# beautifulv0id/Convex-2D-GPU-Collision-Detection

Hardware: AMD Instinct MI355X
Metric: sat_pair_tests_per_s (higher is better)
Workload: dtype f32

## Files before the change

convex-2d-gpu-collision-detection_amd/csrc/c2d_math.hpp:

```cpp
#pragma once

#include <hip/hip_runtime.h>
#include <stdint.h>

namespace c2d {

#define C2D_DEV __device__ __forceinline__

C2D_DEV float fma_(float a, float b, float c) { return __builtin_fmaf(a, b, c); }

C2D_DEV float log_(float u)
{
    uint32_t t = __float_as_uint(u) - 0x3f2aaaabu;
    int32_t e = (int32_t)t >> 23;
    float m = __uint_as_float((t & 0x007fffffu) + 0x3f2aaaabu);
    float f = m - 1.0f;
    float q = -0x1.04cba2p-3f;
    q = fma_(q, f, 0x1.19bbe2p-3f);
    q = fma_(q, f, -0x1.f483fap-4f);
    q = fma_(q, f, 0x1.1fd494p-3f);
    q = fma_(q, f, -0x1.55913ep-3f);
    q = fma_(q, f, 0x1.99bffep-3f);
    q = fma_(q, f, -0x1.ffff28p-3f);
    q = fma_(q, f, 0x1.55552cp-2f);
    q = fma_(q, f, -0x1.000000p-1f);
    float s = f * f;
    float r = fma_(s, q, f);
    return fma_((float)e, 0x1.62e430p-1f, r);
}

C2D_DEV float sqrt_normal_range(float x)
{
    const float s = __builtin_amdgcn_sqrtf(x);
    const float s_dn = __uint_as_float(__float_as_uint(s) - 1u);
    const float s_up = __uint_as_float(__float_as_uint(s) + 1u);
    const float r_dn = fma_(-s_dn, s, x);
    const float r_up = fma_(-s_up, s, x);
    float r = r_dn <= 0.0f ? s_dn : s;
    r = r_up > 0.0f ? s_up : r;
    return r;
}

C2D_DEV void quadrant_rotate(int q, float sn, float cs, float& s_out, float& c_out)
{
    float a = (q & 1) ? cs : sn;
    float b = (q & 1) ? sn : cs;
    uint32_t s_sign = ((uint32_t)q & 2u) << 30;
    uint32_t c_sign = (((uint32_t)q + 1u) & 2u) << 30;
    s_out = __uint_as_float(__float_as_uint(a) ^ s_sign);
    c_out = __uint_as_float(__float_as_uint(b) ^ c_sign);
}

C2D_DEV void sincos_(float x, float& s_out, float& c_out)
{
    float k = __builtin_rintf(x * 0x1.45f306p-1f);
    float r = fma_(k, -0x1.920000p+0f, x);
    r = fma_(k, -0x1.fb4000p-12f, r);
    r = fma_(k, -0x1.4442d2p-24f, r);
    float z = r * r;
    float sp = 0x1.6dac7ap-19f;
    sp = fma_(sp, z, -0x1.a01376p-13f);
    sp = fma_(sp, z, 0x1.11110ep-7f);
    sp = fma_(sp, z, -0x1.555556p-3f);
    float sn = fma_(z * r, sp, r);
    float cp = -0x1.2476a8p-22f;
    cp = fma_(cp, z, 0x1.a012bap-16f);
    cp = fma_(cp, z, -0x1.6c16bcp-10f);
    cp = fma_(cp, z, 0x1.555556p-5f);
    cp = fma_(cp, z, -0x1.000000p-1f);
    float cs = fma_(z, cp, 1.0f);
    float kc = __builtin_amdgcn_fmed3f(k, -1073741824.0f, 1073741824.0f);
    int q = (int)kc;
    quadrant_rotate(q, sn, cs, s_out, c_out);
}

C2D_DEV void sincos_u32(uint32_t y, float& s_out, float& c_out)
{
    int q = (int)(y >> 30);
    uint32_t fr = y & 0x3fffffffu;
    bool swap = fr > 0x20000000u;
    fr = swap ? 0x40000000u - fr : fr;
    float x = (float)(int32_t)fr * 0x1p-30f;
    float z = x * x;
    float p = 0x1.4bb0a6p-13f;
    p = fma_(p, z, -0x1.32ca4ap-8f);
    p = fma_(p, z, 0x1.466bbap-4f);
    p = fma_(p, z, -0x1.4abbcep-1f);
    p = fma_(p, z, 0x1.921fb6p+0f);
    float sn = p * x;
    float c = 0x1.d99986p-11f;
    c = fma_(c, z, -0x1.55c4e6p-6f);
    c = fma_(c, z, 0x1.03c1dap-2f);
    c = fma_(c, z, -0x1.3bd3ccp+0f);
    c = fma_(c, z, 1.0f);
    float sn2 = swap ? c : sn;
    float cs2 = swap ? sn : c;
    quadrant_rotate(q, sn2, cs2, s_out, c_out);
}

struct U4 { uint32_t x, y, z, w; };

C2D_DEV U4 philox4x32_10(uint32_t c0, uint32_t c1, uint32_t c2, uint32_t c3, uint32_t k0, uint32_t k1)
{
#pragma unroll
    for (int round = 0; round < 10; round++) {
        uint64_t p0 = (uint64_t)0xD2511F53u * c0;
        uint64_t p1 = (uint64_t)0xCD9E8D57u * c2;
        uint32_t n0 = __builtin_amdgcn_bitop3_b32((uint32_t)(p1 >> 32), c1, k0, 0x96);
        uint32_t n1 = (uint32_t)p1;
        uint32_t n2 = __builtin_amdgcn_bitop3_b32((uint32_t)(p0 >> 32), c3, k1, 0x96);
        uint32_t n3 = (uint32_t)p0;
        c0 = n0; c1 = n1; c2 = n2; c3 = n3;
        k0 += 0x9E3779B9u;
        k1 += 0xBB67AE85u;
    }
    return U4{c0, c1, c2, c3};
}

C2D_DEV U4 philox_block(uint64_t seed, uint64_t scene, uint64_t sample, uint32_t j)
{
    uint64_t blk = 2 * sample + j;
    return philox4x32_10((uint32_t)blk, (uint32_t)(blk >> 32), (uint32_t)scene, (uint32_t)(scene >> 32),
                         (uint32_t)seed, (uint32_t)(seed >> 32));
}

C2D_DEV U4 philox_draw_block(uint64_t seed, uint64_t scene, uint64_t group, uint32_t b)
{
    uint64_t blk = 8 * group + b;
    return philox4x32_10((uint32_t)blk, (uint32_t)(blk >> 32), (uint32_t)scene, (uint32_t)(scene >> 32),
                         (uint32_t)seed, (uint32_t)(seed >> 32));
}

C2D_DEV uint32_t u4_word(const U4& v, int j) { return j == 0 ? v.x : (j == 1 ? v.y : (j == 2 ? v.z : v.w)); }

C2D_DEV void box_muller(uint32_t x, uint32_t y, float& n0, float& n1)
{
    float u = fma_((float)x, 0x1p-32f, 0x1p-33f);
    float rad = sqrt_normal_range(-2.0f * log_(u));
    float sn, cs;
    sincos_u32(y, sn, cs);
    n0 = sn * rad;
    n1 = cs * rad;
}


#ifndef C2D_FMAD
#define C2D_FMAD 0
#endif
C2D_DEV float dot2(float a, float x, float b, float y)
{
#if C2D_FMAD == 1
    return fma_(a, x, b * y);
#elif C2D_FMAD == 2
    return fma_(b, y, a * x);
#else
    return a * x + b * y;
#endif
}

C2D_DEV void rect_from_half_extents(float hx, float hy, float c, float s, float dx, float dy, float (&r)[8])
{
#if C2D_FMAD == 1
    float b = s * hy, q = c * hy;
    float t1 = fma_(c, hx, b), t2 = fma_(c, hx, -b), t3 = fma_(s, hx, q), t4 = fma_(s, hx, -q);
#elif C2D_FMAD == 2
    float a = c * hx, p = s * hx;
    float t1 = fma_(s, hy, a), t2 = fma_(-s, hy, a), t3 = fma_(c, hy, p), t4 = fma_(-c, hy, p);
#else
    float a = c * hx, b = s * hy, p = s * hx, q = c * hy;
    float t1 = a + b, t2 = a - b, t3 = p + q, t4 = p - q;
#endif
    r[0] = dx - t2;
    r[1] = dy - t3;
    r[2] = t1 + dx;
    r[3] = t4 + dy;
    r[4] = t2 + dx;
    r[5] = t3 + dy;
    r[6] = dx - t1;
    r[7] = dy - t4;
}

C2D_DEV void poly_minmax(float nx, float ny, float x, float y, float& mn, float& mx)
{
    const float p = nx * x + ny * y;
    mn = __builtin_fminf(mn, p);
    mx = __builtin_fmaxf(mx, p);
}

C2D_DEV float min4(float a, float b, float c, float d) { return __builtin_fminf(__builtin_fminf(a, b), __builtin_fminf(c, d)); }
C2D_DEV float max4(float a, float b, float c, float d) { return __builtin_fmaxf(__builtin_fmaxf(a, b), __builtin_fmaxf(c, d)); }

C2D_DEV bool first_projections_ordered(float p1_first, float p2_first) { return !__builtin_isunordered(p1_first, p2_first); }

C2D_DEV bool axis_separates(float ax, float ay, const float (&r1)[8], const float (&r2)[8])
{
    float p10 = dot2(ax, r1[0], ay, r1[1]), p11 = dot2(ax, r1[2], ay, r1[3]);
    float p12 = dot2(ax, r1[4], ay, r1[5]), p13 = dot2(ax, r1[6], ay, r1[7]);
    float p20 = dot2(ax, r2[0], ay, r2[1]), p21 = dot2(ax, r2[2], ay, r2[3]);
    float p22 = dot2(ax, r2[4], ay, r2[5]), p23 = dot2(ax, r2[6], ay, r2[7]);
    float min1 = min4(p10, p11, p12, p13), max1 = max4(p10, p11, p12, p13);
    float min2 = min4(p20, p21, p22, p23), max2 = max4(p20, p21, p22, p23);
    return ((max1 < min2) || (max2 < min1)) && first_projections_ordered(p10, p20);
}

C2D_DEV bool rect_collide(const float (&r1)[8], const float (&r2)[8])
{
    bool sep = false;
#pragma unroll
    for (int i = 0; i < 4; i++) {
        float ax = r1[(2 * i + 2) & 7] - r1[2 * i];
        float ay = r1[(2 * i + 3) & 7] - r1[2 * i + 1];
        sep |= axis_separates(ax, ay, r1, r2);
    }
#pragma unroll
    for (int i = 0; i < 4; i++) {
        float ax = r2[(2 * i + 2) & 7] - r2[2 * i];
        float ay = r2[(2 * i + 3) & 7] - r2[2 * i + 1];
        sep |= axis_separates(ax, ay, r1, r2);
    }
    return !sep;
}

C2D_DEV bool rect_collide_certified(const float (&r1)[8], const float (&r2)[8], bool& thin)
{
    float cmax = __builtin_fabsf(r1[0]);
#pragma unroll
    for (int k = 1; k < 8; k++) cmax = __builtin_fmaxf(cmax, __builtin_fabsf(r1[k]));
#pragma unroll
    for (int k = 0; k < 8; k++) cmax = __builtin_fmaxf(cmax, __builtin_fabsf(r2[k]));
    const float c2 = (2.0f + 0x1p-7f) * cmax, c3 = (8.0f + 0x1p-5f) * 0x1p-24f * cmax;
    bool sep = false, uneasy = !(cmax < 0x1p61f);
#pragma unroll
    for (int which = 0; which < 2; which++) {
        const float (&r)[8] = which == 0 ? r1 : r2;
#pragma unroll
        for (int i = 0; i < 2; i++) {
            const float ax = r[2 * i + 2] - r[2 * i], ay = r[2 * i + 3] - r[2 * i + 1];
            const float bx = r[(2 * i + 6) & 7] - r[2 * i + 4], by = r[(2 * i + 7) & 7] - r[2 * i + 5];
            const float p10 = dot2(ax, r1[0], ay, r1[1]), p11 = dot2(ax, r1[2], ay, r1[3]);
            const float p12 = dot2(ax, r1[4], ay, r1[5]), p13 = dot2(ax, r1[6], ay, r1[7]);
            const float p20 = dot2(ax, r2[0], ay, r2[1]), p21 = dot2(ax, r2[2], ay, r2[3]);
            const float p22 = dot2(ax, r2[4], ay, r2[5]), p23 = dot2(ax, r2[6], ay, r2[7]);
            const float min1 = min4(p10, p11, p12, p13), max1 = max4(p10, p11, p12, p13);
            const float min2 = min4(p20, p21, p22, p23), max2 = max4(p20, p21, p22, p23);
            sep |= ((max1 < min2) || (max2 < min1)) && first_projections_ordered(p10, p20);
            const float need = fma_(__builtin_fabsf(ax) + __builtin_fabsf(ay), c3, (__builtin_fabsf(ax + bx) + __builtin_fabsf(ay + by)) * c2) + 1e-36f;
            uneasy |= !((max2 - min1 >= need) && (max1 - min2 >= need));
        }
    }
    thin = !sep && uneasy;
    return !sep;
}

}
```

convex-2d-gpu-collision-detection_amd/csrc/c2d_sat.hip:

```cpp
#include "c2d_internal.hpp"
#include "c2d_math.hpp"
#include "c2d_count.hpp"
#include "c2d_wave.hpp"

namespace c2d {

struct Planes16 { const float* p[16]; };
struct Planes10 { const float* p[10]; };
struct Planes8 { float* p[8]; };

constexpr int kBlock = 256;
constexpr int kWideBlock = 64;
constexpr int kMaxBlocks = kMaxGrid;


template <int PAIRS, class Build>
C2D_DEV uint32_t collide_pairs(Build build)
{
    uint32_t bits = 0;
    bool any_thin = false;
#pragma unroll
    for (int e = 0; e < PAIRS; e++) {
        float r1[8], r2[8];
        build(e, Plain{}, r1, r2);
        bool thin;
        bits |= (rect_collide_certified(r1, r2, thin) ? 1u : 0u) << e;
        any_thin |= thin;
    }
    if (__ballot(any_thin) != 0ull) {
        bits = 0;
#pragma unroll
        for (int e = 0; e < PAIRS; e++) {
            float r1[8], r2[8];
            build(e, Laundered{}, r1, r2);
            bits |= (rect_collide(r1, r2) ? 1u : 0u) << e;
        }
    }
    return bits;
}

C2D_DEV uint32_t bits_to_bytes4(uint32_t b) { return (b & 1u) | ((b & 2u) << 7) | ((b & 4u) << 14) | ((b & 8u) << 21); }

template <int VEC, int BLOCK>
__global__ __launch_bounds__(BLOCK, (VEC == 4 ? 5 : 1)) void sat_rect_verts_kernel(Planes16 P, size_t first, size_t n_groups,
                                                                uint8_t* __restrict__ out,
                                                                unsigned long long* __restrict__ d_count, CountWs words)
{
    uint32_t my_count = 0;
    const size_t stride = (size_t)gridDim.x * BLOCK;
    for (size_t g = (size_t)blockIdx.x * BLOCK + threadIdx.x; g < n_groups; g += stride) {
        if constexpr (VEC == 4) {
            f32x4 v[16];
#pragma unroll
            for (int k = 0; k < 16; k++) v[k] = __builtin_nontemporal_load(reinterpret_cast<const f32x4*>(P.p[k]) + g);
            const uint32_t packed = bits_to_bytes4(collide_pairs<4>([&v](int e, auto how, float (&r1)[8], float (&r2)[8]) {
#pragma unroll
                for (int k = 0; k < 8; k++) {
                    r1[k] = launder(v[k][e], how);
                    r2[k] = launder(v[8 + k][e], how);
                }
            }));
            my_count += (uint32_t)__popc(packed);
            __builtin_nontemporal_store(packed, reinterpret_cast<uint32_t*>(out) + g);
        } else {
            const size_t i = first + g;
            float r1[8], r2[8];
#pragma unroll
            for (int k = 0; k < 8; k++) {
                r1[k] = P.p[k][i];
                r2[k] = P.p[8 + k][i];
            }
            uint32_t c = rect_collide(r1, r2) ? 1u : 0u;
            out[i] = (uint8_t)c;
            my_count += c;
        }
    }
    if (d_count) wave_count_arrive(my_count, d_count, words);
}

__global__ __launch_bounds__(64) void sat_rect_verts_mask4_kernel(Planes16 P, size_t n_groups, unsigned long long* __restrict__ mask,
                                                                  unsigned long long* __restrict__ d_count,
                                                                  CountWs words)
{
    const uint32_t lane = threadIdx.x;
    const size_t g = (size_t)blockIdx.x * 64 + lane;
    uint32_t nib = 0;
    if (g < n_groups) {
        f32x4 v[16];
#pragma unroll
        for (int k = 0; k < 16; k++) v[k] = __builtin_nontemporal_load(reinterpret_cast<const f32x4*>(P.p[k]) + g);
        nib = collide_pairs<4>([&v](int e, auto how, float (&r1)[8], float (&r2)[8]) {
#pragma unroll
            for (int k = 0; k < 8; k++) {
                r1[k] = launder(v[k][e], how);
                r2[k] = launder(v[8 + k][e], how);
            }
        });
    }
    const uint32_t sh = 4u * (lane & 15u);
    uint32_t lo = sh < 32u ? nib << sh : 0u, hi = sh >= 32u ? nib << (sh - 32u) : 0u;
#pragma unroll
    for (int off = 1; off < 16; off <<= 1) {
        lo |= (uint32_t)__shfl_xor((int)lo, off, 64);
        hi |= (uint32_t)__shfl_xor((int)hi, off, 64);
    }
    if ((lane & 15u) == 0 && g < n_groups) __builtin_nontemporal_store(((unsigned long long)hi << 32) | lo, mask + ((size_t)blockIdx.x * 4 + (lane >> 4)));
    if (d_count) wave_count_arrive((uint32_t)__popc(nib), d_count, words);
}

__global__ __launch_bounds__(kBlock) void sat_rect_verts_mask1_kernel(Planes16 P, size_t first, size_t n, unsigned long long* __restrict__ mask,
                                                                      unsigned long long* __restrict__ d_count,
                                                                      CountWs words)
{
    uint32_t my_count = 0;
    const size_t stride = (size_t)gridDim.x * kBlock;
    const size_t n_round = (n + 63) / 64 * 64;
    for (size_t i = first + (size_t)blockIdx.x * kBlock + threadIdx.x; i < n_round; i += stride) {
        uint32_t c = 0;
        if (i < n) {
            float r1[8], r2[8];
#pragma unroll
            for (int k = 0; k < 8; k++) {
                r1[k] = P.p[k][i];
                r2[k] = P.p[8 + k][i];
            }
            c = rect_collide(r1, r2) ? 1u : 0u;
        }
        const unsigned long long b = __ballot(c != 0);
        if ((threadIdx.x & 63) == 0) mask[i >> 6] = b;
        my_count += c;
    }
    if (d_count) wave_count_arrive(my_count, d_count, words);
}

template <bool OUT16>
__global__ __launch_bounds__(64) void sat_rect_aos_kernel(const float* __restrict__ r1s, const float* __restrict__ r2s,
                                                         size_t n, uint8_t* __restrict__ out,
                                                         unsigned long long* __restrict__ d_count,
                                                         CountWs words)
{
    constexpr int kChunks = 256;
    __shared__ __attribute__((aligned(16))) f32x4 tile[2][kChunks];
    const int lane = threadIdx.x;
    uint32_t my_count = 0;
    const size_t n_tiles = (n + 127) / 128;
    for (size_t t = blockIdx.x; t < n_tiles; t += gridDim.x) {
        const size_t p0 = t * 128;
        const size_t chunks = (n - p0 < 128 ? n - p0 : 128) * 2;
        const f32x4* a = reinterpret_cast<const f32x4*>(r1s) + 2 * p0;
        const f32x4* b = reinterpret_cast<const f32x4*>(r2s) + 2 * p0;
        const f32x4 zero = {0.f, 0.f, 0.f, 0.f};
        f32x4 va[4], vb[4];
#pragma unroll
        for (int k = 0; k < 4; k++) {
            const size_t c = (size_t)(64 * k + lane);
            va[k] = c < chunks ? __builtin_nontemporal_load(a + c) : zero;
            vb[k] = c < chunks ? __builtin_nontemporal_load(b + c) : zero;
        }
#pragma unroll
        for (int k = 0; k < 4; k++) {
            tile[0][64 * k + lane] = va[k];
            tile[1][64 * k + lane] = vb[k];
        }
        wave_lds_sync();
        f32x4 pa[4], pb[4];
#pragma unroll
        for (int c = 0; c < 4; c++) {
            pa[c] = tile[0][4 * lane + c];
            pb[c] = tile[1][4 * lane + c];
        }
        const uint32_t bits = collide_pairs<2>([&pa, &pb](int e, auto how, float (&r1)[8], float (&r2)[8]) {
#pragma unroll
            for (int k = 0; k < 8; k++) {
                r1[k] = launder(pa[2 * e + k / 4][k % 4], how);
                r2[k] = launder(pb[2 * e + k / 4][k % 4], how);
            }
        });
        const uint32_t packed = (bits & 1u) | ((bits & 2u) << 7);
        const size_t i = p0 + 2 * (size_t)lane;
        if (i + 1 < n) {
            if constexpr (OUT16) {
                *reinterpret_cast<uint16_t*>(out + i) = (uint16_t)packed;
            } else {
                out[i] = (uint8_t)(packed & 1u);
                out[i + 1] = (uint8_t)(packed >> 8);
            }
            my_count += (uint32_t)__popc(packed);
        } else if (i < n) {
            out[i] = (uint8_t)(packed & 1u);
            my_count += packed & 1u;
        }
        wave_lds_sync();
    }
    if (d_count) wave_count_arrive(my_count, d_count, words);
}

C2D_DEV bool pose_pair_closed_form(const float (&v)[10], bool& thin)
{
    float s1, c1, s2, c2;
    sincos_(v[4], s1, c1);
    sincos_(v[9], s2, c2);
    const float hw = __builtin_fabsf(v[2] / 2), hh = __builtin_fabsf(v[3] / 2), hx = __builtin_fabsf(v[7] / 2), hy = __builtin_fabsf(v[8] / 2);
    const float q1 = fma_(c1, c2, s1 * s2), q2 = fma_(c1, s2, -(s1 * c2));
    const float ex = v[5] - v[0], ey = v[6] - v[1];
    const float t1 = fma_(c1, ex, s1 * ey), t2 = fma_(c1, ey, -(s1 * ex));
    const float t3 = fma_(c2, ex, s2 * ey), t4 = fma_(c2, ey, -(s2 * ex));
    const float a1 = __builtin_fabsf(q1), a2 = __builtin_fabsf(q2);
    const float g1 = __builtin_fabsf(t1) - fma_(hx, a1, fma_(hy, a2, hw));
    const float g2 = __builtin_fabsf(t2) - fma_(hx, a2, fma_(hy, a1, hh));
    const float g3 = __builtin_fabsf(t3) - fma_(hw, a1, fma_(hh, a2, hx));
    const float g4 = __builtin_fabsf(t4) - fma_(hw, a2, fma_(hh, a1, hy));
    const float C = __builtin_fmaxf(__builtin_fmaxf(__builtin_fabsf(v[0]), __builtin_fabsf(v[1])) + (hw + hh),
                                    __builtin_fmaxf(__builtin_fabsf(v[5]), __builtin_fabsf(v[6])) + (hx + hy)) * (1.0f + 0x1p-10f);
    const float uc = (0x1p-24f * (1.0f + 0x1p-10f)) * C, k64 = 64.0f * uc, k20 = (20.0f * uc) * C;
    const float z1 = g1 * hw, z2 = g2 * hh, z3 = g3 * hx, z4 = g4 * hy;
    const float m1 = fma_(k64, hw, k20), m2 = fma_(k64, hh, k20), m3 = fma_(k64, hx, k20), m4 = fma_(k64, hy, k20);
    const float over = __builtin_fmaxf(__builtin_fmaxf(z1 - m1, z2 - m2), __builtin_fmaxf(z3 - m3, z4 - m4));
    const float under = __builtin_fmaxf(__builtin_fmaxf(z1 + m1, z2 + m2), __builtin_fmaxf(z3 + m3, z4 + m4));
    const float all = (g1 + g2) + (g3 + g4);
    const float hmin = __builtin_fminf(__builtin_fminf(hw, hh), __builtin_fminf(hx, hy));
    const bool regular = (C < 1e15f) & (hmin >= 1e-12f) & (__builtin_fabsf(all) < 1e37f);
    const bool sep = over > 0.0f, col = under < 0.0f;
    thin = !(regular & (sep | col));
    return col;
}

C2D_DEV void pose_pair_rects(const float (&v)[10], float (&r1)[8], float (&r2)[8])
{
    float s, c;
    sincos_(v[4], s, c);
    rect_from_half_extents(v[2] / 2, v[3] / 2, c, s, v[0], v[1], r1);
    sincos_(v[9], s, c);
    rect_from_half_extents(v[7] / 2, v[8] / 2, c, s, v[5], v[6], r2);
}

C2D_DEV uint32_t pose_pair_collides(const float (&v)[10])
{
    float r1[8], r2[8];
    pose_pair_rects(v, r1, r2);
    return rect_collide(r1, r2) ? 1u : 0u;
}

template <int VEC, int BLOCK>
__global__ __launch_bounds__(BLOCK, (VEC == 4 ? 5 : 1)) void sat_rect_pose_kernel(Planes10 P, size_t first, size_t n_groups,
                                                              uint8_t* __restrict__ out,
                                                              unsigned long long* __restrict__ d_count,
                                                              CountWs words)
{
    uint32_t my_count = 0;
    const size_t stride = (size_t)gridDim.x * BLOCK;
    for (size_t g = (size_t)blockIdx.x * BLOCK + threadIdx.x; g < n_groups; g += stride) {
        if constexpr (VEC == 4) {
            f32x4 q[10];
#pragma unroll
            for (int k = 0; k < 10; k++) q[k] = __builtin_nontemporal_load(reinterpret_cast<const f32x4*>(P.p[k]) + g);
            uint32_t bits = 0;
#pragma unroll
            for (int e = 0; e < 4; e++) {
                float v[10];
#pragma unroll
                for (int k = 0; k < 10; k++) v[k] = q[k][e];
                bool thin;
                uint32_t hit = pose_pair_closed_form(v, thin) ? 1u : 0u;
                if (__ballot(thin) != 0ull) {
                    hit = collide_pairs<1>([&q, e](int, auto, float (&r1)[8], float (&r2)[8]) {
                        float w[10];
#pragma unroll
                        for (int k = 0; k < 10; k++) w[k] = launder(q[k][e], Laundered{});
                        pose_pair_rects(w, r1, r2);
                    });
                }
                bits |= hit << e;
            }
            const uint32_t packed = bits_to_bytes4(bits);
            my_count += (uint32_t)__popc(packed);
            __builtin_nontemporal_store(packed, reinterpret_cast<uint32_t*>(out) + g);
        } else {
            const size_t i = first + g;
            float v[10];
#pragma unroll
            for (int k = 0; k < 10; k++) v[k] = P.p[k][i];
            const uint32_t hit = pose_pair_collides(v);
            out[i] = (uint8_t)hit;
            my_count += hit;
        }
    }
    if (d_count) wave_count_arrive(my_count, d_count, words);
}

__global__ __launch_bounds__(kBlock) void rects_from_poses_kernel(const float* __restrict__ cx, const float* __restrict__ cy,
                                                                  const float* __restrict__ w, const float* __restrict__ h,
                                                                  const float* __restrict__ th, size_t n, Planes8 O)
{
    const size_t stride = (size_t)gridDim.x * kBlock;
    for (size_t i = (size_t)blockIdx.x * kBlock + threadIdx.x; i < n; i += stride) {
        float r[8], s, c;
        sincos_(th[i], s, c);
        rect_from_half_extents(w[i] / 2, h[i] / 2, c, s, cx[i], cy[i], r);
#pragma unroll
        for (int k = 0; k < 8; k++) O.p[k][i] = r[k];
    }
}

__global__ __launch_bounds__(kWideBlock) void rects_from_poses4_kernel(const float* __restrict__ cx, const float* __restrict__ cy,
                                                                       const float* __restrict__ w, const float* __restrict__ h,
                                                                       const float* __restrict__ th, size_t n_groups, Planes8 O)
{
    const size_t stride = (size_t)gridDim.x * kWideBlock;
    for (size_t g = (size_t)blockIdx.x * kWideBlock + threadIdx.x; g < n_groups; g += stride) {
        const f32x4 vcx = __builtin_nontemporal_load(reinterpret_cast<const f32x4*>(cx) + g);
        const f32x4 vcy = __builtin_nontemporal_load(reinterpret_cast<const f32x4*>(cy) + g);
        const f32x4 vw = __builtin_nontemporal_load(reinterpret_cast<const f32x4*>(w) + g);
        const f32x4 vh = __builtin_nontemporal_load(reinterpret_cast<const f32x4*>(h) + g);
        const f32x4 vt = __builtin_nontemporal_load(reinterpret_cast<const f32x4*>(th) + g);
        f32x4 o[8];
#pragma unroll
        for (int e = 0; e < 4; e++) {
            float r[8], s, c;
            sincos_(vt[e], s, c);
            rect_from_half_extents(vw[e] / 2, vh[e] / 2, c, s, vcx[e], vcy[e], r);
#pragma unroll
            for (int k = 0; k < 8; k++) o[k][e] = r[k];
        }
#pragma unroll
        for (int k = 0; k < 8; k++) __builtin_nontemporal_store(o[k], reinterpret_cast<f32x4*>(O.p[k]) + g);
    }
}

static inline bool aligned_to(const void* p, size_t a) { return (reinterpret_cast<uintptr_t>(p) & (a - 1)) == 0; }

}

using namespace c2d;

extern "C" {

int c2d_rects_from_poses(c2d_ctx* ctx, const float* d_cx, const float* d_cy, const float* d_w, const float* d_h,
                         const float* d_theta, size_t n, float* const d_out_planes[8], c2d_stream stream)
{
    if (!ctx) return C2D_ERR_INVALID_ARG;
    if (n == 0) return C2D_OK;
    if (!d_cx || !d_cy || !d_w || !d_h || !d_theta || !d_out_planes) return fail_arg(ctx, "c2d_rects_from_poses: NULL plane");
    Planes8 O;
    for (int k = 0; k < 8; k++) {
        if (!d_out_planes[k]) return fail_arg(ctx, "c2d_rects_from_poses: NULL output plane");
        O.p[k] = d_out_planes[k];
    }
    DeviceGuard g(ctx->device);
    bool wide = aligned_to(d_cx, 16) && aligned_to(d_cy, 16) && aligned_to(d_w, 16) && aligned_to(d_h, 16) && aligned_to(d_theta, 16);
    for (int k = 0; k < 8; k++) wide = wide && aligned_to(O.p[k], 16);
    const size_t n4 = wide ? n / 4 : 0;
    if (n4) {
        hipLaunchKernelGGL(rects_from_poses4_kernel, dim3(grid_for(n4, kWideBlock, kMaxBlocks)), dim3(kWideBlock), 0, (hipStream_t)stream, d_cx, d_cy,
                           d_w, d_h, d_theta, n4, O);
        C2D_LAUNCH_CHECK(ctx);
    }
    const size_t rest = n - 4 * n4;
    if (rest) {
        Planes8 T;
        for (int k = 0; k < 8; k++) T.p[k] = O.p[k] + 4 * n4;
        hipLaunchKernelGGL(rects_from_poses_kernel, dim3(grid_for(rest, kBlock, ctx->prop.multiProcessorCount * 8)), dim3(kBlock), 0,
                           (hipStream_t)stream, d_cx + 4 * n4, d_cy + 4 * n4, d_w + 4 * n4, d_h + 4 * n4, d_theta + 4 * n4, rest, T);
        C2D_LAUNCH_CHECK(ctx);
    }
    return C2D_OK;
}

int c2d_sat_rect_pairs_verts(c2d_ctx* ctx, const float* const d_planes[16], size_t n, uint8_t* d_out,
                             unsigned long long* d_count, c2d_stream stream)
{
    if (!ctx) return C2D_ERR_INVALID_ARG;
    if (n == 0) return C2D_OK;
    if (!d_planes || !d_out) return fail_arg(ctx, "c2d_sat_rect_pairs_verts: NULL argument");
    Planes16 P;
    bool wide = aligned_to(d_out, 4);
    for (int k = 0; k < 16; k++) {
        if (!d_planes[k]) return fail_arg(ctx, "c2d_sat_rect_pairs_verts: NULL plane");
        P.p[k] = d_planes[k];
        wide = wide && aligned_to(d_planes[k], 16);
    }
    DeviceGuard g(ctx->device);
    hipStream_t s = (hipStream_t)stream;
    if (int rc = workspace_acquire(ctx, s, d_count != nullptr)) return rc;
    const size_t n4 = wide ? n / 4 : 0;
    if (n4) {
        const int grid = grid_for(n4, kWideBlock, kMaxBlocks);
        hipLaunchKernelGGL((sat_rect_verts_kernel<4, kWideBlock>), dim3(grid), dim3(kWideBlock), 0, s, P, (size_t)0, n4, d_out,
                           d_count, workspace_count_ticket(ctx, s, (size_t)grid * (kWideBlock / 64), d_count != nullptr));
        C2D_LAUNCH_CHECK(ctx);
    }
    const size_t rest = n - 4 * n4;
    if (rest) {
        const int grid = grid_for(rest, kBlock, kMaxBlocks);
        hipLaunchKernelGGL((sat_rect_verts_kernel<1, kBlock>), dim3(grid), dim3(kBlock), 0, s, P, 4 * n4, rest, d_out, d_count,
                           workspace_count_ticket(ctx, s, (size_t)grid * (kBlock / 64), d_count != nullptr));
        C2D_LAUNCH_CHECK(ctx);
    }
    return C2D_OK;
}

int c2d_sat_rect_pairs_verts_mask(c2d_ctx* ctx, const float* const d_planes[16], size_t n, unsigned long long* d_mask,
                                  unsigned long long* d_count, c2d_stream stream)
{
    if (!ctx) return C2D_ERR_INVALID_ARG;
    if (n == 0) return C2D_OK;
    if (!d_planes || !d_mask) return fail_arg(ctx, "c2d_sat_rect_pairs_verts_mask: NULL argument");
    if (!aligned_to(d_mask, 8)) return fail_arg(ctx, "c2d_sat_rect_pairs_verts_mask: the mask must be 8-byte aligned");
    Planes16 P;
    bool wide = true;
    for (int k = 0; k < 16; k++) {
        if (!d_planes[k]) return fail_arg(ctx, "c2d_sat_rect_pairs_verts_mask: NULL plane");
        P.p[k] = d_planes[k];
        wide = wide && aligned_to(d_planes[k], 16);
    }
    DeviceGuard g(ctx->device);
    hipStream_t s = (hipStream_t)stream;
    if (int rc = workspace_acquire(ctx, s, d_count != nullptr)) return rc;
    size_t done = 0;
    while (wide && n - done >= 64) {
        size_t words_left = (n - done) / 64;
        if (words_left > (size_t)kMaxBlocks * 4) words_left = (size_t)kMaxBlocks * 4;
        Planes16 Q;
        for (int k = 0; k < 16; k++) Q.p[k] = P.p[k] + done;
        const size_t groups = words_left * 16;
        hipLaunchKernelGGL(sat_rect_verts_mask4_kernel, dim3((unsigned)((groups + 63) / 64)), dim3(64), 0, s, Q, groups, d_mask + done / 64, d_count,
                           workspace_count_ticket(ctx, s, (groups + 63) / 64, d_count != nullptr));
        C2D_LAUNCH_CHECK(ctx);
        done += words_left * 64;
    }
    if (done < n) {
        const int grid = grid_for(n - done, kBlock, kMaxBlocks);
        hipLaunchKernelGGL(sat_rect_verts_mask1_kernel, dim3(grid), dim3(kBlock), 0, s, P, done, n, d_mask, d_count,
                           workspace_count_ticket(ctx, s, (size_t)grid * (kBlock / 64), d_count != nullptr));
        C2D_LAUNCH_CHECK(ctx);
    }
    return C2D_OK;
}

int c2d_sat_rect_pairs_aos(c2d_ctx* ctx, const float* d_r1, const float* d_r2, size_t n, uint8_t* d_out,
                           unsigned long long* d_count, c2d_stream stream)
{
    if (!ctx) return C2D_ERR_INVALID_ARG;
    if (n == 0) return C2D_OK;
    if (!d_r1 || !d_r2 || !d_out) return fail_arg(ctx, "c2d_sat_rect_pairs_aos: NULL argument");
    if (!aligned_to(d_r1, 16) || !aligned_to(d_r2, 16)) return fail_arg(ctx, "c2d_sat_rect_pairs_aos: rectangle arrays must be 16-byte aligned");
    DeviceGuard g(ctx->device);
    if (int rc = workspace_acquire(ctx, (hipStream_t)stream, d_count != nullptr)) return rc;
    const int grid = grid_for(n, 128, kMaxBlocks);
    const CountWs ws = workspace_count_ticket(ctx, (hipStream_t)stream, (size_t)grid, d_count != nullptr);
    if (aligned_to(d_out, 2))
        hipLaunchKernelGGL(sat_rect_aos_kernel<true>, dim3(grid), dim3(64), 0, (hipStream_t)stream, d_r1, d_r2, n, d_out, d_count, ws);
    else
        hipLaunchKernelGGL(sat_rect_aos_kernel<false>, dim3(grid), dim3(64), 0, (hipStream_t)stream, d_r1, d_r2, n, d_out, d_count, ws);
    C2D_LAUNCH_CHECK(ctx);
    return C2D_OK;
}

int c2d_sat_rect_pairs_pose(c2d_ctx* ctx, const float* const d_pose_planes[10], size_t n, uint8_t* d_out,
                            unsigned long long* d_count, c2d_stream stream)
{
    if (!ctx) return C2D_ERR_INVALID_ARG;
    if (n == 0) return C2D_OK;
    if (!d_pose_planes || !d_out) return fail_arg(ctx, "c2d_sat_rect_pairs_pose: NULL argument");
    Planes10 P;
    bool wide = aligned_to(d_out, 4);
    for (int k = 0; k < 10; k++) {
        if (!d_pose_planes[k]) return fail_arg(ctx, "c2d_sat_rect_pairs_pose: NULL plane");
        P.p[k] = d_pose_planes[k];
        wide = wide && aligned_to(d_pose_planes[k], 16);
    }
    DeviceGuard g(ctx->device);
    hipStream_t s = (hipStream_t)stream;
    if (int rc = workspace_acquire(ctx, s, d_count != nullptr)) return rc;
    const size_t n4 = wide ? n / 4 : 0;
    if (n4) {
        const int grid = grid_for(n4, kWideBlock, kMaxBlocks);
        hipLaunchKernelGGL((sat_rect_pose_kernel<4, kWideBlock>), dim3(grid), dim3(kWideBlock), 0, s, P, (size_t)0, n4, d_out,
                           d_count, workspace_count_ticket(ctx, s, (size_t)grid * (kWideBlock / 64), d_count != nullptr));
        C2D_LAUNCH_CHECK(ctx);
    }
    const size_t rest = n - 4 * n4;
    if (rest) {
        const int grid = grid_for(rest, kBlock, kMaxBlocks);
        hipLaunchKernelGGL((sat_rect_pose_kernel<1, kBlock>), dim3(grid), dim3(kBlock), 0, s, P, 4 * n4, rest, d_out, d_count,
                           workspace_count_ticket(ctx, s, (size_t)grid * (kBlock / 64), d_count != nullptr));
        C2D_LAUNCH_CHECK(ctx);
    }
    return C2D_OK;
}

}
```

Before: 95.60 billion.

## Replace certified SAT projection test with center-gap formulation and simplify pose fallback

Replaces the per-axis min/max projection certified test with a rectangle gap test. It uses center differences, edge-vector dot products and rounding-error margins, so each axis needs far fewer dot products and min/max operations. The pose kernel fallback now calls pose_pair_collides directly on laundered inputs instead of going through collide_pairs. The new error bounds must remain sound, and they may send more pairs down the thin/exact fallback path.

```diff
diff --git a/convex-2d-gpu-collision-detection_amd/csrc/c2d_math.hpp b/convex-2d-gpu-collision-detection_amd/csrc/c2d_math.hpp
--- a/convex-2d-gpu-collision-detection_amd/csrc/c2d_math.hpp
+++ b/convex-2d-gpu-collision-detection_amd/csrc/c2d_math.hpp
@@ -221,35 +221,39 @@
     return !sep;
 }
 
-C2D_DEV bool rect_collide_certified(const float (&r1)[8], const float (&r2)[8], bool& thin)
-{
-    float cmax = __builtin_fabsf(r1[0]);
-#pragma unroll
-    for (int k = 1; k < 8; k++) cmax = __builtin_fmaxf(cmax, __builtin_fabsf(r1[k]));
-#pragma unroll
-    for (int k = 0; k < 8; k++) cmax = __builtin_fmaxf(cmax, __builtin_fabsf(r2[k]));
-    const float c2 = (2.0f + 0x1p-7f) * cmax, c3 = (8.0f + 0x1p-5f) * 0x1p-24f * cmax;
-    bool sep = false, uneasy = !(cmax < 0x1p61f);
-#pragma unroll
-    for (int which = 0; which < 2; which++) {
-        const float (&r)[8] = which == 0 ? r1 : r2;
-#pragma unroll
-        for (int i = 0; i < 2; i++) {
-            const float ax = r[2 * i + 2] - r[2 * i], ay = r[2 * i + 3] - r[2 * i + 1];
-            const float bx = r[(2 * i + 6) & 7] - r[2 * i + 4], by = r[(2 * i + 7) & 7] - r[2 * i + 5];
-            const float p10 = dot2(ax, r1[0], ay, r1[1]), p11 = dot2(ax, r1[2], ay, r1[3]);
-            const float p12 = dot2(ax, r1[4], ay, r1[5]), p13 = dot2(ax, r1[6], ay, r1[7]);
-            const float p20 = dot2(ax, r2[0], ay, r2[1]), p21 = dot2(ax, r2[2], ay, r2[3]);
-            const float p22 = dot2(ax, r2[4], ay, r2[5]), p23 = dot2(ax, r2[6], ay, r2[7]);
-            const float min1 = min4(p10, p11, p12, p13), max1 = max4(p10, p11, p12, p13);
-            const float min2 = min4(p20, p21, p22, p23), max2 = max4(p20, p21, p22, p23);
-            sep |= ((max1 < min2) || (max2 < min1)) && first_projections_ordered(p10, p20);
-            const float need = fma_(__builtin_fabsf(ax) + __builtin_fabsf(ay), c3, (__builtin_fabsf(ax + bx) + __builtin_fabsf(ay + by)) * c2) + 1e-36f;
-            uneasy |= !((max2 - min1 >= need) && (max1 - min2 >= need));
-        }
-    }
-    thin = !sep && uneasy;
-    return !sep;
-}
-
-}
+
+C2D_DEV float dotf(float px, float py, float qx, float qy) { return fma_(px, qx, py * qy); }
+
+C2D_DEV bool rect_gap_certified(const float (&r1)[8], const float (&r2)[8], bool& thin)
+{
+    const float a1x = r1[2] - r1[0], a1y = r1[3] - r1[1], b1x = r1[6] - r1[0], b1y = r1[7] - r1[1];
+    const float a2x = r2[2] - r2[0], a2y = r2[3] - r2[1], b2x = r2[6] - r2[0], b2y = r2[7] - r2[1];
+    const float s1x = r1[0] + r1[4], s1y = r1[1] + r1[5], s2x = r2[0] + r2[4], s2y = r2[1] + r2[5];
+    const float e1 = __builtin_fabsf(s1x - (r1[2] + r1[6])) + __builtin_fabsf(s1y - (r1[3] + r1[7]));
+    const float e2 = __builtin_fabsf(s2x - (r2[2] + r2[6])) + __builtin_fabsf(s2y - (r2[3] + r2[7]));
+    const float dx = s2x - s1x, dy = s2y - s1y;
+    float C = __builtin_fabsf(r1[0]);
+#pragma unroll
+    for (int k = 1; k < 8; k++) C = __builtin_fmaxf(C, __builtin_fabsf(r1[k]));
+#pragma unroll
+    for (int k = 0; k < 8; k++) C = __builtin_fmaxf(C, __builtin_fabsf(r2[k]));
+    const float a1b1 = __builtin_fabsf(dotf(a1x, a1y, b1x, b1y)), a2b2 = __builtin_fabsf(dotf(a2x, a2y, b2x, b2y));
+    const float a1a2 = __builtin_fabsf(dotf(a1x, a1y, a2x, a2y)), a1b2 = __builtin_fabsf(dotf(a1x, a1y, b2x, b2y));
+    const float b1a2 = __builtin_fabsf(dotf(b1x, b1y, a2x, a2y)), b1b2 = __builtin_fabsf(dotf(b1x, b1y, b2x, b2y));
+    const float g1 = __builtin_fabsf(dotf(a1x, a1y, dx, dy)) - ((dotf(a1x, a1y, a1x, a1y) + a1b1) + (a1a2 + a1b2));
+    const float g2 = __builtin_fabsf(dotf(b1x, b1y, dx, dy)) - ((dotf(b1x, b1y, b1x, b1y) + a1b1) + (b1a2 + b1b2));
+    const float g3 = __builtin_fabsf(dotf(a2x, a2y, dx, dy)) - ((dotf(a2x, a2y, a2x, a2y) + a2b2) + (a1a2 + b1a2));
+    const float g4 = __builtin_fabsf(dotf(b2x, b2y, dx, dy)) - ((dotf(b2x, b2y, b2x, b2y) + a2b2) + (a1b2 + b1b2));
+    const float m0 = fma_(3.02f, e1 + e2, (120.0f * 0x1p-24f) * C);
+    const float c4 = 4.02f * C, cc = fma_((33.0f * 0x1p-24f) * C, C, 1e-36f);
+    const float n1 = fma_(c4, e1, cc), n2 = fma_(c4, e2, cc);
+    const float m1 = fma_(__builtin_fabsf(a1x) + __builtin_fabsf(a1y), m0, n1), m2 = fma_(__builtin_fabsf(b1x) + __builtin_fabsf(b1y), m0, n1);
+    const float m3 = fma_(__builtin_fabsf(a2x) + __builtin_fabsf(a2y), m0, n2), m4 = fma_(__builtin_fabsf(b2x) + __builtin_fabsf(b2y), m0, n2);
+    const float over = __builtin_fmaxf(__builtin_fmaxf(g1 - m1, g2 - m2), __builtin_fmaxf(g3 - m3, g4 - m4));
+    const float under = __builtin_fmaxf(__builtin_fmaxf(g1 + m1, g2 + m2), __builtin_fmaxf(g3 + m3, g4 + m4));
+    const bool col = under < 0.0f;
+    thin = !((C < 0x1p61f) & ((over > 0.0f) | col));
+    return col;
+}
+
+}
diff --git a/convex-2d-gpu-collision-detection_amd/csrc/c2d_sat.hip b/convex-2d-gpu-collision-detection_amd/csrc/c2d_sat.hip
--- a/convex-2d-gpu-collision-detection_amd/csrc/c2d_sat.hip
+++ b/convex-2d-gpu-collision-detection_amd/csrc/c2d_sat.hip
@@ -24,7 +24,7 @@
         float r1[8], r2[8];
         build(e, Plain{}, r1, r2);
         bool thin;
-        bits |= (rect_collide_certified(r1, r2, thin) ? 1u : 0u) << e;
+        bits |= (rect_gap_certified(r1, r2, thin) ? 1u : 0u) << e;
         any_thin |= thin;
     }
     if (__ballot(any_thin) != 0ull) {
@@ -263,12 +263,10 @@
                 bool thin;
                 uint32_t hit = pose_pair_closed_form(v, thin) ? 1u : 0u;
                 if (__ballot(thin) != 0ull) {
-                    hit = collide_pairs<1>([&q, e](int, auto, float (&r1)[8], float (&r2)[8]) {
-                        float w[10];
-#pragma unroll
-                        for (int k = 0; k < 10; k++) w[k] = launder(q[k][e], Laundered{});
-                        pose_pair_rects(w, r1, r2);
-                    });
+                    float w[10];
+#pragma unroll
+                    for (int k = 0; k < 10; k++) w[k] = launder(q[k][e], Laundered{});
+                    hit = pose_pair_collides(w);
                 }
                 bits |= hit << e;
             }
```

New measurement: 96.64 billion, median of 6. +1.1%, better.
